# JanLohse/raw2film

Hardware: AMD Instinct MI355X
Metric: megapixels/sec full film pipeline (neg+print+grain+halation+MTF), 100MP frame (higher is better)
Workload: dtype f32 (pointwise stages, grain) + f64 (FFT stencils; the MTF's scratch images are complex64)

## Files before the change

### raw2film_amd/context.py

```python

from __future__ import annotations

import ctypes as C

import numpy as np

from . import _lib

LOG_EPS = 1e-6
LUT3D_SCALE = 0.25


class R2FError(RuntimeError):
    pass


def _host_f32(a) -> np.ndarray:
    return np.ascontiguousarray(np.asarray(a, dtype=np.float32))


class HipContext:
    def __init__(self, device: int = 0, lib_path: str | None = None):
        import torch

# ... 432 lines not shown
        self._check(self._lib.r2f_decode_u16(self._h, image_u16.data_ptr(), int(image_u16.shape[0]), int(image_u16.shape[1]),
                                             int(image_u16.shape[2]), float(np.float32(divisor)), float(np.float32(factor)),
                                             out.data_ptr(), self._stream()))
        return out

    def blit_rgba8(self, image_f32, dst_rgba, transform: dict):
        torch = self._torch
        if not (image_f32.is_cuda and image_f32.dtype == torch.float32 and image_f32.is_contiguous() and image_f32.dim() == 3
                and image_f32.shape[2] == 3):
            raise ValueError("blit_rgba8 needs a contiguous float32 (H, W, 3) CUDA tensor")
        if not (dst_rgba.is_cuda and dst_rgba.dtype == torch.uint8 and dst_rgba.is_contiguous() and dst_rgba.dim() == 3
                and dst_rgba.shape[2] == 4):
            raise ValueError("blit_rgba8 needs a contiguous uint8 (h, w, 4) CUDA destination")
        self._same_device(image_f32, "image")
        self._same_device(dst_rgba, "destination")
        t = _lib.Blit(transform["scale_x"], transform["scale_y"], transform["offset_x"], transform["offset_y"],
                      transform["canvas_min_x"], transform["canvas_min_y"], transform["canvas_max_x"], transform["canvas_max_y"],
                      (C.c_float * 3)(*transform["canvas_color"]))
        self._check(self._lib.r2f_blit_rgba8(self._h, image_f32.data_ptr(), int(image_f32.shape[0]), int(image_f32.shape[1]),
                                             dst_rgba.data_ptr(), int(dst_rgba.shape[0]), int(dst_rgba.shape[1]), C.byref(t),
                                             self._stream()))
        return dst_rgba

    def histogram_render(self, counts, mix_table, height: int, target=None):
        torch = self._torch
        mix = np.ascontiguousarray(np.asarray(mix_table, dtype=np.uint8).reshape(8, 4))
        image = torch.empty((int(height), 256, 4), dtype=torch.uint8, device=self.device)
        if not (isinstance(counts, torch.Tensor) and counts.is_cuda and counts.dtype in (torch.int32, torch.uint32)
                and tuple(counts.shape) == (3, 256)):
            raise ValueError("histogram_render needs the (3, 256) int32 CUDA counts of histogram_counts")
        self._same_device(counts, "counts")
        counts = counts.contiguous()
        if target is not None and not (target.is_cuda and target.dtype == torch.uint8 and target.is_contiguous() and target.dim() == 3
                                       and target.shape[2] == 4):
            raise ValueError("histogram_render needs a contiguous uint8 (h, w, 4) CUDA target")
        if target is not None:
            self._same_device(target, "target")
        self._check(self._lib.r2f_histogram_render(
            self._h, counts.data_ptr(), mix.ctypes.data, int(height), image.data_ptr(),
            target.data_ptr() if target is not None else None, int(target.shape[0]) if target is not None else 0,
            int(target.shape[1]) if target is not None else 0, self._stream()))
        return image

    def stencil_stats(self, which: int):
        out = (C.c_int * 24)()
        self._check(self._lib.r2f_stencil_stats(self._h, int(which), out))
        keys = ("entries", "rowsteps", "phases", "sym", "kh", "kw", "q")
        stats = []
        for c in range(3):
            d = dict(zip(keys, out[8 * c:8 * c + 7]))
            word = out[8 * c + 7]
            d["unrolled"] = (d["sym"] >> 1) & 0x7F
            d["separable"] = (d["sym"] >> 8) & 1
            d["sym"] &= 1
            d["fft"] = word & 1
            dims = (word >> 1) & 0x1FFFFFFF
            d["window"] = (dims // 4096, dims % 4096) if dims else None
            d["real_spectrum"] = (word >> 30) & 1
            stats.append(d)
        return stats

    def stream_copy(self, src, dst):
        nbytes = src.numel() * src.element_size()
        if dst.numel() * dst.element_size() != nbytes or not (src.is_cuda and dst.is_cuda and src.is_contiguous() and dst.is_contiguous()):
            raise ValueError("stream_copy needs two contiguous CUDA tensors of the same size in bytes")
        self._same_device(src, "source")
        self._same_device(dst, "destination")
        self._check(self._lib.r2f_stream_copy(self._h, src.data_ptr(), dst.data_ptr(), nbytes, self._stream()))

    def kernel_timing(self, cls: int):
        ms, n, b = C.c_double(), C.c_int(), C.c_double()
        self._check(self._lib.r2f_kernel_timing(self._h, int(cls), C.byref(ms), C.byref(n), C.byref(b)))
        return ms.value, n.value, b.value

    def histogram_counts(self, image_u8):
        torch = self._torch
        if not (image_u8.is_cuda and image_u8.dtype == torch.uint8 and image_u8.is_contiguous() and image_u8.dim() == 3
                and image_u8.shape[2] == 3):
            raise ValueError("histogram_counts needs a contiguous uint8 (H, W, 3) CUDA tensor")
        self._same_device(image_u8, "image")
        counts = torch.empty((3, 256), dtype=torch.int32, device=self.device)
        self._check(self._lib.r2f_histogram_u8(self._h, image_u8.data_ptr(), int(image_u8.shape[0]), int(image_u8.shape[1]),
                                               counts.data_ptr(), self._stream()))
        return counts

    def jpeg_bound_bytes(self, H: int, W: int, subsampling: int = 2) -> int:
        if int(subsampling) == 2:
            return int(self._lib.r2f_jpeg_bound_bytes(int(H), int(W)))
        return int(self._lib.r2f_jpeg_bound_bytes_ex(int(H), int(W), int(subsampling)))

    def jpeg_bound_bytes_opts(self, H: int, W: int, quality: int, subsampling: int = 2, optimize: bool = False,
                              progressive: bool = False) -> int:
        opts = _lib.JpegOpts(int(quality), int(subsampling), 1 if optimize else 0, 1 if progressive else 0)
        return int(self._lib.r2f_jpeg_bound_bytes_opts(C.byref(opts), int(H), int(W)))

    def jpeg_encode(self, image_u8, quality: int, subsampling: int = 2, optimize: bool = False, progressive: bool = False):
        torch = self._torch
        if not (isinstance(image_u8, torch.Tensor) and image_u8.is_cuda and image_u8.dtype == torch.uint8 and image_u8.dim() == 3
                and image_u8.shape[2] == 3 and image_u8.stride(2) == 1 and image_u8.stride(1) == 3):
            raise ValueError("jpeg_encode needs a uint8 (H, W, 3) CUDA tensor with packed pixels (row stride free)")
        self._same_device(image_u8, "image")
        H, W = int(image_u8.shape[0]), int(image_u8.shape[1])
        bound = (self.jpeg_bound_bytes_opts(H, W, quality, subsampling, optimize, True) if progressive else
                 self.jpeg_bound_bytes(H, W, subsampling))
        if bound == 0:
            raise ValueError(f"jpeg_encode: a JPEG holds 1 .. 65535 pixels per side, got {H} x {W} (subsampling {subsampling})")
# ... 56 lines not shown
```

### raw2film_amd/csrc/r2f_api.hip

```cpp
#include <hip/hip_runtime.h>

#include <cmath>
#include <cstdarg>
#include <cstdio>
#include <cstring>
#include <string>
#include <algorithm>
#include <vector>

#include "../../include/r2f.h"
#include "r2f_launch.h"
#include "r2f_jpeg.h"
#include "r2f_plan.h"

using namespace r2f;

namespace {

struct DeviceBuf {
    void* p = nullptr;
    size_t bytes = 0;
    void release() {
        if (p) (void)hipFree(p);
        p = nullptr;
// ... 33 lines not shown
    DevCurve grain_lut{};
    StencilSet stencil[3];
    struct TileOrder {
        int gx = 0, gy = 0;
        DeviceBuf buf;
    } tile_order[4];
    int tile_order_next = 0;
    static constexpr int kFftShapes = 6;
    static int fft_shape_index(int ny, int nx) { return (ny == 512 ? 3 : 0) + (nx == 256 ? 0 : (nx == 512 ? 1 : 2)); }
    DeviceBuf fft_tw, fft_kf[3][3][kFftShapes], fft_s1, fft_kimg;
    bool fft_kf_valid[3][3][kFftShapes] = {};
    int fft_kf_dims[3][3] = {{0, 0, 0}, {0, 0, 0}, {0, 0, 0}};
    int fft_last_real[3][3] = {{0, 0, 0}, {0, 0, 0}, {0, 0, 0}};
    int opt_fft_window = 0;
    int opt_fft_window_max = 512;
    int opt_fft_window_rows = 0;
    int opt_timing = 0;
    std::vector<std::pair<hipEvent_t, hipEvent_t>> timing_ev[6];
    double timing_bytes[6] = {0, 0, 0, 0, 0, 0};
    int opt_fft = 1;
    int opt_fft_min_taps = 400;
    hipStream_t fft_stream[4] = {nullptr, nullptr, nullptr, nullptr};
    hipEvent_t fft_ev_in = nullptr, fft_ev_out[4] = {nullptr, nullptr, nullptr, nullptr};
    int opt_fft_streams = 2;
    int opt_fft_even = 1;
    int opt_fft_batch = 192;
    int opt_fft_s32 = 1 << R2F_KERNEL_MTF;
    int opt_fft_s96 = 0;
    int opt_fft_s96_auto = 1;
    float curve_slope_max = 0.f;
    bool frame_dyn_armed = false;
    bool capturing = false;
    int opt_fft_epi_lds = 1;
    int opt_fft_real = 1;
    int opt_fft_mixed_sign = 1;
    int opt_fft_cols_walk = 1;
    int cu_count = 0;
    bool fft_kf_real[3][3][kFftShapes] = {};
    DeviceBuf lanczos_buf;
    DeviceBuf lanczos_f32_buf;
    int lanczos_key[4] = {0, 0, 0, 0};
    int opt_xcd_band = 0;
    int opt_variant = -1;
    int opt_xcd_remap = 2;
    int opt_ablate = 0;
    int opt_sym = 1;
    DeviceBuf grain_fixed_w;
    bool grain_fixed_valid = false;
    int grain_fixed_r = 0, grain_fixed_same = 0;
    int opt_grain_fixed = 1;
    bool grain_sep = false;
    float grain_sep_u[3][19] = {}, grain_sep_v[3][10] = {};
    int opt_grain_sep = 1;
    DeviceBuf stencil_fixed_w[3];
    bool stencil_fixed_valid[3] = {false, false, false};
    int opt_stencil_fixed = 1;
    int opt_front_fast = 1;
    int opt_front_blocks = 6;
    int opt_lds_kb = 80;
    DeviceBuf frame_buf;
    DeviceBuf range_tiles, dyn_flags;
    int tiles_tyn = 0, tiles_txn = 0;
    int dyn_flags_ppc = 0;
    struct RenderGraph {
        const void* in = nullptr;
        int in_layout = 0;
        float* out_f32 = nullptr;
        uint8_t* out_u8 = nullptr;
        int H = 0, W = 0;
        void* workspace = nullptr;
        r2f_params p{};
        hipGraph_t graph = nullptr;
        hipGraphExec_t exec = nullptr;
        hipEvent_t done = nullptr;
        uint64_t last_use = 0;
        bool never = false;
        bool dyn_armed = false;
    };
    std::vector<RenderGraph> graphs;
    struct RetiredGraph {
        hipGraph_t graph;
        hipGraphExec_t exec;
        hipEvent_t done;
    };
    std::vector<RetiredGraph> retired;
    uint64_t graphs_generation = 0;
    uint64_t graph_clock = 0;
    RenderGraph warm;
    bool warm_valid = false;
    std::vector<RenderGraph> seen;
    hipStream_t cap_stream = nullptr;
    int opt_render_graph = 1;
    uint64_t stat_replays = 0, stat_captures = 0, stat_eager = 0, stat_dropped = 0;
    DeviceBuf jpeg_scratch;
    struct JpegRows {
        bool open = false;
        int H = 0, W = 0, next_y = 0;
        int sampling = 2, header_len = 0;
        uint8_t* out = nullptr;
        uint64_t* out_len = nullptr;
    } jpeg_rows;
    DeviceBuf jpeg_carry;
    DeviceBuf jpeg_freq;
};

namespace {
// ... 691 lines not shown
        return R2F_OK;
    }
    if (!strcmp(name, "stencil_lds_kb")) {
        if (value < 8 || value > 160) return fail(ctx, R2F_EINVAL, "stencil_lds_kb must be in [8, 160]");
        ctx->opt_lds_kb = value;
        return R2F_OK;
    }
    if (!strcmp(name, "stencil_sym")) {
        ctx->opt_sym = value ? 1 : 0;
        return R2F_OK;
    }
    if (!strcmp(name, "stencil_ablate")) {
        ctx->opt_ablate = value;
        return R2F_OK;
    }
    if (!strcmp(name, "kernel_timing")) {
        ctx->opt_timing = value & 7;
        return R2F_OK;
    }
    if (!strcmp(name, "stencil_fft")) {
        ctx->opt_fft = value ? 1 : 0;
        return R2F_OK;
    }
    if (!strcmp(name, "stencil_fft_window")) {
        if (value != 0 && value != 256 && value != 512 && value != 1024) return fail(ctx, R2F_EINVAL, "stencil_fft_window must be 0, 256, 512 or 1024");
        ctx->opt_fft_window = value;
        return R2F_OK;
    }
    if (!strcmp(name, "stencil_fft_window_max")) {
        if (value != 256 && value != 512 && value != 1024) return fail(ctx, R2F_EINVAL, "stencil_fft_window_max must be 256, 512 or 1024");
        ctx->opt_fft_window_max = value;
        return R2F_OK;
    }
    if (!strcmp(name, "stencil_fft_even_batches")) {
        ctx->opt_fft_even = value ? 1 : 0;
        return R2F_OK;
    }
    if (!strcmp(name, "stencil_fixed")) {
        ctx->opt_stencil_fixed = value ? 1 : 0;
        return R2F_OK;
    }
    if (!strcmp(name, "grain_fixed")) {
        ctx->opt_grain_fixed = value ? 1 : 0;
        return R2F_OK;
    }
    if (!strcmp(name, "front_fast")) {
        ctx->opt_front_fast = value ? 1 : 0;
        return R2F_OK;
    }
    if (!strcmp(name, "grain_separable")) {
        ctx->opt_grain_sep = value ? 1 : 0;
        return R2F_OK;
    }
    if (!strcmp(name, "front_blocks_per_cu")) {
        if (value < 1 || value > 64) return fail(ctx, R2F_EINVAL, "front_blocks_per_cu must be in [1, 64]");
        ctx->opt_front_blocks = value;
        return R2F_OK;
    }
    if (!strcmp(name, "stencil_fft_window_rows")) {
        if (value != 0 && value != 256 && value != 512) return fail(ctx, R2F_EINVAL, "stencil_fft_window_rows must be 0, 256 or 512");
        ctx->opt_fft_window_rows = value;
        return R2F_OK;
    }
    if (!strcmp(name, "stencil_fft_min_taps")) {
        ctx->opt_fft_min_taps = value;
        return R2F_OK;
    }
    if (!strcmp(name, "stencil_fft_streams")) {
        if (value < 1 || value > 4) return fail(ctx, R2F_EINVAL, "stencil_fft_streams must be in [1, 4]");
        ctx->opt_fft_streams = value;
        return R2F_OK;
    }
    if (!strcmp(name, "stencil_fft_cols_walk")) {
        ctx->opt_fft_cols_walk = value ? 1 : 0;
        return R2F_OK;
    }
    if (!strcmp(name, "stencil_fft_mixed_sign")) {
        ctx->opt_fft_mixed_sign = value ? 1 : 0;
        return R2F_OK;
    }
    if (!strcmp(name, "stencil_fft_real_spectrum")) {
        ctx->opt_fft_real = value ? 1 : 0;
        return R2F_OK;
    }
    if (!strcmp(name, "stencil_fft_epilogue_lds")) {
        ctx->opt_fft_epi_lds = value ? 1 : 0;
        return R2F_OK;
    }
    if (!strcmp(name, "stencil_fft_scratch96_auto")) {
        ctx->opt_fft_s96_auto = value ? 1 : 0;
        return R2F_OK;
    }
    if (!strcmp(name, "stencil_fft_scratch96")) {
        if (value < 0 || value > 7) return fail(ctx, R2F_EINVAL, "stencil_fft_scratch96 is a mask over the three stencils (0..7)");
        ctx->opt_fft_s96 = value;
        return R2F_OK;
    }
    if (!strcmp(name, "stencil_fft_scratch32")) {
        if (value < 0 || value > 7) return fail(ctx, R2F_EINVAL, "stencil_fft_scratch32 is a mask over the three stencils (0..7)");
        ctx->opt_fft_s32 = value;
        return R2F_OK;
    }
    if (!strcmp(name, "stencil_fft_batch")) {
        if (value < 1) return fail(ctx, R2F_EINVAL, "stencil_fft_batch must be >= 1");
        ctx->opt_fft_batch = value;
        return R2F_OK;
// ... 248 lines not shown
    if (!ctx || !p) return R2F_EINVAL;
    R2F_GUARD(ctx);
    return run_stencil(ctx, R2F_KERNEL_MTF, din, dout, y0, y1, W, H_global, 0, 0.f, static_cast<hipStream_t>(stream));
}

int r2f_stage_stencil(r2f_ctx* ctx, int which, const r2f_planes* src, const r2f_planes* dst, int y0, int y1, int W,
                      int H_global, void* stream) {
    if (!ctx) return R2F_EINVAL;
    R2F_GUARD(ctx);
    if (which < 0 || which > 2) return fail(ctx, R2F_EINVAL, "stencil: which must be 0..2");
    return run_stencil(ctx, which, src, dst, y0, y1, W, H_global, 0, 0.f, static_cast<hipStream_t>(stream));
}

int r2f_kernel_timing(r2f_ctx* ctx, int cls, double* total_ms, int* launches, double* bytes) {
    if (!ctx || cls < 0 || cls > 5 || !total_ms || !launches || !bytes) return R2F_EINVAL;
    R2F_GUARD(ctx);
    double sum = 0.0;
    for (auto& ev : ctx->timing_ev[cls]) {
        R2F_HIP(ctx, hipEventSynchronize(ev.second));
        float ms = 0.f;
        R2F_HIP(ctx, hipEventElapsedTime(&ms, ev.first, ev.second));
        sum += ms;
        (void)hipEventDestroy(ev.first);
        (void)hipEventDestroy(ev.second);
    }
    *total_ms = sum;
    *launches = (int)ctx->timing_ev[cls].size();
    *bytes = ctx->timing_bytes[cls];
    ctx->timing_ev[cls].clear();
    ctx->timing_bytes[cls] = 0.0;
    return R2F_OK;
}

int r2f_stencil_stats(r2f_ctx* ctx, int which, int* out) {
    if (!ctx || !out) return R2F_EINVAL;
    R2F_GUARD(ctx);
    if (which < 0 || which > 2) return fail(ctx, R2F_EINVAL, "stencil: which must be 0..2");
    StencilSet& set = ctx->stencil[which];
    if (!set.present) return fail(ctx, R2F_EINVAL, "stencil %d not set (r2f_set_kernel)", which);
    if (!set.built_q) {
        const StencilVariant& sv = kStencilVariants[ctx->opt_variant >= 0 ? ctx->opt_variant : 0];
        int rc = ensure_stencil(ctx, which, sv.Q, sv.TW(), sv.TH(), (size_t)ctx->opt_lds_kb * 1024, which == 2);
        if (rc) return rc;
    }
    for (int c = 0; c < 3; ++c) {
        const DevStencil& d = set.dev[c];
        int* o = out + 8 * c;
        const int all[3] = {0, 1, 2};
        const int fr = which == R2F_KERNEL_GRAIN ? (ctx->opt_grain_fixed ? fixed_stencil_radius(set, all, 3, 9) : 0)
                                                 : (ctx->opt_stencil_fixed && ctx->opt_variant <= 0 && !fft_eligible(ctx, set, c)
                                                        ? fixed_stencil_radius(set, &c, 1, kFixedMaxR)
                                                        : 0);
        const int sep = which == R2F_KERNEL_GRAIN && fr && ctx->grain_fixed_valid && ctx->grain_sep && ctx->opt_grain_sep;
        o[0] = d.n_entries, o[1] = d.n_rowsteps, o[2] = d.n_phases, o[3] = d.sym | (fr << 1) | (sep << 8);
        o[4] = d.kh, o[5] = d.kw, o[6] = set.built_q;
        o[7] = fft_eligible(ctx, set, c) ? 1 | (ctx->fft_kf_dims[which][c] << 1) | (ctx->fft_last_real[which][c] << 30) : 0;
    }
    return R2F_OK;
}

static bool burn_geometry(const r2f_params* p, int H, int W, int* h_lo, int* w_lo) { return plan::burn_geometry(p->burn_cell, H, W, h_lo, w_lo); }

static int ensure_grain_fixed(r2f_ctx* ctx) {
    if (ctx->grain_fixed_valid) return R2F_OK;
    StencilSet& set = ctx->stencil[R2F_KERNEL_GRAIN];
    ctx->grain_fixed_valid = true;
    const int chans[3] = {0, 1, 2};
    ctx->grain_fixed_r = fixed_stencil_radius(set, chans, 3, 9);
    ctx->grain_sep = false;
    if (!ctx->grain_fixed_r) return R2F_OK;
    bool same = false;
    const std::vector<float> w = fixed_stencil_weights(set, ctx->grain_fixed_r, kTailQ, &same);
    ctx->grain_fixed_same = same ? 1 : 0;
    ctx->grain_sep = plan::separable_taps(taps_of(set), ctx->grain_fixed_r, ctx->grain_sep_u, ctx->grain_sep_v);
    return upload(ctx, ctx->grain_fixed_w, w.data(), w.size() * sizeof(float));
}

static int run_tail(r2f_ctx* ctx, const r2f_params* p, const r2f_planes* density, const r2f_planes* planes_out,
                    const float* burn_map, float* out_f32, uint8_t* out_u8, int out_gy0, int y0, int y1, int W, int H_global,
                    void* stream, const r2f_planes* gfield = nullptr) {
    if (y1 <= y0) return R2F_OK;
    const bool field_only = density == nullptr && planes_out != nullptr;
    if (field_only) {
        static const r2f_planes none = {nullptr, 0, 0, 0};
        density = &none;
    }
    const bool to_planes = planes_out != nullptr;
    if (W <= 0 || y0 < 0 || y1 > H_global || (!to_planes && y0 < out_gy0)) return fail(ctx, R2F_EINVAL, "tail: bad geometry");
    if (!to_planes && !out_f32 && !out_u8) return fail(ctx, R2F_EINVAL, "tail: no output buffer");
    if (!to_planes && !ctx->lut3d.tex) return fail(ctx, R2F_EINVAL, "output LUT not set (r2f_set_lut3d)");
    int rc = field_only ? R2F_OK : check_rows(ctx, "tail src", density, y0, y1);
    if (rc) return rc;
    TailArgs a;
    memset(&a, 0, sizeof a);
    a.src = to_dev(density);
    a.out_f32 = out_f32;
    a.out_u8 = out_u8;
    a.out_gy0 = out_gy0;
    a.y0 = y0;
    a.y1 = y1;
    a.W = W;
    a.H_global = H_global;
    a.grain = (p->flags & R2F_F_GRAIN) ? 1 : 0;
    if (gfield) {
        if (!a.grain) return fail(ctx, R2F_EINVAL, "tail: a grain field was passed but the grain flag is off");
        rc = check_rows(ctx, "grain field", gfield, y0, y1);
        if (rc) return rc;
// ... 6 lines not shown
    a.mono = (p->flags & R2F_F_GRAIN_MONO) ? 1 : 0;
    a.frame = static_cast<const FrameParams*>(ctx->frame_buf.p);
    a.lut3d = ctx->lut3d;
    a.lut3d_scale = p->lut3d_scale;
    a.lut3d_mode = p->lut3d_mode;
    bool vec = field_only ? true : planes_vec_ok(density, W);
    if (gfield) vec = vec && planes_vec_ok(gfield, W);
    if (to_planes) {
        if (!a.grain) return fail(ctx, R2F_EINVAL, "grain stage called with the grain flag off");
        rc = check_rows(ctx, "grain dst", planes_out, y0, y1);
        if (rc) return rc;
        if (!field_only && planes_overlap(density, planes_out, W) &&
            !(density->data == planes_out->data && density->plane_stride == planes_out->plane_stride && density->gy0 == planes_out->gy0))
            return fail(ctx, R2F_EINVAL, "grain: source and destination planes overlap without being the same buffer");
        a.to_planes = field_only ? 2 : 1;
        a.dst = to_dev(planes_out);
        vec = vec && planes_vec_ok(planes_out, W);
    } else {
        vec = vec && (!out_f32 || aligned16(out_f32)) && (!out_u8 || (reinterpret_cast<uintptr_t>(out_u8) & 3u) == 0);
        if (burn_map) {
            if (a.grain || a.has_gfield)
                return fail(ctx, R2F_EINVAL, "tail with a burn map: apply the grain first (r2f_stage_grain) and clear R2F_F_GRAIN");
            int h_lo, w_lo;
            if (!burn_geometry(p, H_global, W, &h_lo, &w_lo)) return fail(ctx, R2F_EINVAL, "burn: bad burn_cell");
            a.burn.map = burn_map;
            a.burn.h_lo = h_lo;
            a.burn.w_lo = w_lo;
            a.burn.h_up = h_lo * p->burn_cell;
            a.burn.w_up = w_lo * p->burn_cell;
            a.burn.zy = a.burn.h_up > 1 ? (double)(h_lo - 1) / (double)(a.burn.h_up - 1) : 0.0;
            a.burn.zx = a.burn.w_up > 1 ? (double)(w_lo - 1) / (double)(a.burn.w_up - 1) : 0.0;
            a.burn.strength = p->burn_strength;
        }
    }
    a.vec = vec ? 1 : 0;
    if (a.grain) {
        if (!ctx->grain_lut.cells) return fail(ctx, R2F_EINVAL, "grain LUT not set (r2f_set_grain_lut)");
        if (!ctx->stencil[R2F_KERNEL_GRAIN].present) {
            const float one = 1.f;
            rc = r2f_set_kernel(ctx, R2F_KERNEL_GRAIN, &one, 1, 1, 1);
            if (rc) return rc;
        }
        rc = ensure_stencil(ctx, R2F_KERNEL_GRAIN, kTailQ, 4 * kTailBX, kTailQ * kTailBY, 0, true);
        if (rc) return rc;
        for (int c = 0; c < 3; ++c) a.gk[c] = ctx->stencil[R2F_KERNEL_GRAIN].dev[c];
        rc = ensure_grain_fixed(ctx);
        if (rc) return rc;
        a.fixed_r = ctx->opt_grain_fixed ? ctx->grain_fixed_r : 0;
        a.fixed_same = ctx->grain_fixed_same;
        a.fixed_w = static_cast<const float*>(ctx->grain_fixed_w.p);
        a.sep = (a.fixed_r && ctx->opt_grain_sep && ctx->grain_sep && (!a.mono || ctx->grain_fixed_same)) ? 1 : 0;
        memcpy(a.sep_u, ctx->grain_sep_u, sizeof a.sep_u);
        memcpy(a.sep_v, ctx->grain_sep_v, sizeof a.sep_v);
        if (tail_lds_bytes(a.gk, a.mono) > kMaxLds)
            return fail(ctx, R2F_ETOOLARGE, "grain stencil %dx%d does not fit the LDS noise tile", a.gk[0].kh, a.gk[0].kw);
        a.grain_lut = ctx->grain_lut;
    }
    if (a.grain && !(p->flags & R2F_F_FRAME_RESIDENT)) {
        rc = write_frame_params(ctx, p, static_cast<hipStream_t>(stream), 0);
        if (rc) return rc;
    }
    R2F_HIP(ctx, launch_tail(a, static_cast<hipStream_t>(stream)));
    return R2F_OK;
}

int r2f_stage_tail(r2f_ctx* ctx, const r2f_params* p, const r2f_planes* density, const float* burn_map, float* out_f32,
                   uint8_t* out_u8, int out_gy0, int y0, int y1, int W, int H_global, void* stream) {
    if (!ctx || !p) return R2F_EINVAL;
    R2F_GUARD(ctx);
    return run_tail(ctx, p, density, nullptr, burn_map, out_f32, out_u8, out_gy0, y0, y1, W, H_global, stream);
}

int r2f_stage_grain_field(r2f_ctx* ctx, const r2f_params* p, const r2f_planes* field, int y0, int y1, int W, int H_global,
                          void* stream) {
    if (!ctx || !p) return R2F_EINVAL;
    R2F_GUARD(ctx);
    if (!field) return fail(ctx, R2F_EINVAL, "grain field: null destination");
    return run_tail(ctx, p, nullptr, field, nullptr, nullptr, nullptr, 0, y0, y1, W, H_global, stream);
}

int r2f_stage_tail_field(r2f_ctx* ctx, const r2f_params* p, const r2f_planes* density, const r2f_planes* field, float* out_f32,
                         uint8_t* out_u8, int out_gy0, int y0, int y1, int W, int H_global, void* stream) {
    if (!ctx || !p) return R2F_EINVAL;
    R2F_GUARD(ctx);
    if (!field) return fail(ctx, R2F_EINVAL, "tail: null grain field");
    return run_tail(ctx, p, density, nullptr, nullptr, out_f32, out_u8, out_gy0, y0, y1, W, H_global, stream, field);
}

int r2f_stage_grain(r2f_ctx* ctx, const r2f_params* p, const r2f_planes* din, const r2f_planes* dout, int y0, int y1, int W,
                    int H_global, void* stream) {
    if (!ctx || !p) return R2F_EINVAL;
    R2F_GUARD(ctx);
    if (!dout) return fail(ctx, R2F_EINVAL, "grain: null destination");
    return run_tail(ctx, p, din, dout, nullptr, nullptr, nullptr, 0, y0, y1, W, H_global, stream);
}

int r2f_stage_burn_sums(r2f_ctx* ctx, const r2f_params* p, const r2f_planes* density, float* cell_sums, int y0, int y1, int W,
                        int H_global, void* stream) {
    if (!ctx || !p) return R2F_EINVAL;
    R2F_GUARD(ctx);
    int h_lo, w_lo;
    if (!cell_sums || !burn_geometry(p, H_global, W, &h_lo, &w_lo)) return fail(ctx, R2F_EINVAL, "burn sums: bad arguments");
    if (y0 < 0 || y1 > H_global || y1 < y0) return fail(ctx, R2F_EINVAL, "burn sums: bad rows");
    if (y1 > y0) {
        int rc = check_rows(ctx, "burn src", density, y0, y1);
        if (rc) return rc;
// ... 728 lines not shown
```

### raw2film_amd/csrc/r2f_kernels.hip

```cpp
#include <algorithm>

#include "r2f_launch.h"

#include "../../include/r2f.h"

#ifndef R2F_CURVE_BATCH3
#define R2F_CURVE_BATCH3 1
#endif

namespace r2f {

const StencilVariant kStencilVariants[kNumStencilVariants] = {
    {0, 32, 16, 4},
    {1, 16, 8, 4},
    {2, 32, 8, 4},
};

__device__ __forceinline__ uint32_t to_u8(float v) {
    float s = fminf(fmaxf(v * 255.0f, 0.0f), 255.0f);
    return (uint32_t)s;
}

__device__ __forceinline__ void emit_hwc(float* out_f32, uint8_t* out_u8, long long orow, int x, int W, int nv, bool vec,
                                         const float (&r)[4], const float (&g)[4], const float (&b)[4]) {
// ... 546 lines not shown
        const int gy = tile_y0 + ty * Q + q;
        if (gy >= a.y1) break;
        float r[4], g[4], b[4];
        if (a.to_planes == 2) {
#pragma unroll
            for (int p = 0; p < 4; ++p) r[p] = G[0][q / 2][p][q & 1], g[p] = G[1][q / 2][p][q & 1], b[p] = G[2][q / 2][p][q & 1];
            store_planes4(a.dst, gy, gx, a.W, nv, vec, r, g, b);
            continue;
        }
#pragma unroll
        for (int p = 0; p < 4; ++p) r[p] = pre_r[q][p], g[p] = pre_g[q][p], b[p] = pre_b[q][p];
#pragma unroll
        for (int p = 0; p < 4; ++p) {
            float ar, ag, ab;
            if (R2F_CURVE_BATCH3) {
                float v3[3] = {r[p], g[p], b[p]};
                if (a.cells_in_lds)
                    curve_eval_batch<3, 3>((const float4*)cells_lds, a.grain_lut, 0, v3);
                else
                    curve_eval_batch<3, 3>(gcells, a.grain_lut, 0, v3);
                ar = v3[0], ag = v3[1], ab = v3[2];
            } else if (a.cells_in_lds) {
                ar = curve_eval_at((const float4*)cells_lds, a.grain_lut, 0, r[p]);
                ag = curve_eval_at((const float4*)cells_lds, a.grain_lut, 1, g[p]);
                ab = curve_eval_at((const float4*)cells_lds, a.grain_lut, 2, b[p]);
            } else {
                ar = curve_eval(a.grain_lut, 0, r[p]);
                ag = curve_eval(a.grain_lut, 1, g[p]);
                ab = curve_eval(a.grain_lut, 2, b[p]);
            }
            r[p] = fmaxf(__fadd_rn(r[p], __fmul_rn(G[0][q / 2][p][q & 1], ar)), 0.f);
            g[p] = fmaxf(__fadd_rn(g[p], __fmul_rn(G[1][q / 2][p][q & 1], ag)), 0.f);
            b[p] = fmaxf(__fadd_rn(b[p], __fmul_rn(G[2][q / 2][p][q & 1], ab)), 0.f);
            if (!a.to_planes && !(R2F_TAIL_EXP & 4)) {
                if (!tetra_nonneg)
                    apply_lut3d(a.lut3d, a.lut3d_scale, a.lut3d_mode, r[p], g[p], b[p]);
                else if (R2F_TAIL_LUT_BATCH == 1)
                    apply_lut3d_tetra_nonneg(a.lut3d, s3, r[p], g[p], b[p]);
                else if ((p + 1) % R2F_TAIL_LUT_BATCH == 0) {
                    constexpr int NB = R2F_TAIL_LUT_BATCH;
                    float rn[NB], gn[NB], bn[NB];
#pragma unroll
                    for (int k = 0; k < NB; ++k) rn[k] = r[p + 1 - NB + k], gn[k] = g[p + 1 - NB + k], bn[k] = b[p + 1 - NB + k];
                    apply_lut3d_tetra_nonneg_batch<NB>(a.lut3d, s3, rn, gn, bn);
#pragma unroll
                    for (int k = 0; k < NB; ++k) r[p + 1 - NB + k] = rn[k], g[p + 1 - NB + k] = gn[k], b[p + 1 - NB + k] = bn[k];
                }
            }
        }
        if (a.to_planes)
            store_planes4(a.dst, gy, gx, a.W, nv, vec, r, g, b);
        else
            emit_hwc(a.out_f32, a.out_u8, gy - a.out_gy0, gx, a.W, nv, vec, r, g, b);
    }
}

__device__ __forceinline__ void area_cell(int d, double scale, int ssize, int& s_first, int& s_last, int& s1, int& s2,
                                          double& w_first, double& w_full, double& w_last) {
    const double f1 = d * scale, f2 = f1 + scale;
    const double cell = fmin(scale, (double)ssize - f1);
    s1 = (int)ceil(f1);
    s2 = min((int)floor(f2), ssize - 1);
    s1 = min(s1, s2);
    w_first = (s1 - f1 > 1e-3) ? (s1 - f1) / cell : 0.0;
    w_full = 1.0 / cell;
    w_last = (f2 - s2 > 1e-3) ? fmin(fmin(f2 - s2, 1.0), cell) / cell : 0.0;
    s_first = max(s1 - 1, 0);
    s_last = s2;
}

__device__ __forceinline__ float area_weight(int s, int s1, int s2, double w_first, double w_full, double w_last) {
    if (s == s1 - 1) return (float)w_first;
    if (s >= s1 && s < s2) return (float)w_full;
    if (s == s2) return (float)w_last;
    return 0.f;
}

__global__ __launch_bounds__(256) void burn_sums_kernel(const BurnSumsArgs a) {
    const int j = blockIdx.x, i = blockIdx.y;
    int ry0, ry1, rs1, rs2, cx0, cx1, cs1, cs2;
    double wyf, wy, wyl, wxf, wx, wxl;
    area_cell(i, (double)a.H_global / a.h_lo, a.H_global, ry0, ry1, rs1, rs2, wyf, wy, wyl);
    area_cell(j, (double)a.W / a.w_lo, a.W, cx0, cx1, cs1, cs2, wxf, wx, wxl);
    const int ra = max(ry0, a.y0), rb = min(ry1, a.y1 - 1);
    const int ncols = cx1 - cx0 + 1;
    const float* green = a.src.data + a.src.plane_stride;
    double acc = 0.0;
    if (rb >= ra) {
        const int n = (rb - ra + 1) * ncols;
        for (int idx = threadIdx.x; idx < n; idx += 256) {
            const int rr = idx / ncols, cc = idx - rr * ncols;
            const int y = ra + rr, x = cx0 + cc;
            const float w = area_weight(y, rs1, rs2, wyf, wy, wyl) * area_weight(x, cs1, cs2, wxf, wx, wxl);
            acc += (double)w * (double)green[(long long)(y - a.src.gy0) * a.W + x];
        }
    }
    __shared__ double red[256];
    red[threadIdx.x] = acc;
    __syncthreads();
    for (int s = 128; s > 0; s >>= 1) {
        if (threadIdx.x < s) red[threadIdx.x] += red[threadIdx.x + s];
        __syncthreads();
    }
    if (threadIdx.x == 0) a.cell_sums[i * a.w_lo + j] = (float)red[0];
}

// ... 371 lines not shown
    if (ldsc) {
        int gy = ((a.blocks_per_cu > 0 ? a.blocks_per_cu : 6) * 256 + gx - 1) / gx;
        if (gy > row_groups) gy = row_groups;
        if (gy < 1) gy = 1;
        launch_k(front_kernel<true>, dim3(gx, gy), block, cell_bytes, s, a);
    } else {
        launch_k(front_kernel<false>, dim3(gx, row_groups), block, 0, s, a);
    }
    return take_launch_status();
}

hipError_t launch_stencil(const StencilArgs& a, int variant, hipStream_t s) {
    if (a.y1 <= a.y0 || a.W <= 0) return hipSuccess;
    const StencilVariant& v = kStencilVariants[variant];
    const size_t lds = stencil_lds_bytes(v, a.st, 3);
    dim3 block(v.BX * v.BY), grid((a.W + v.TW() - 1) / v.TW(), (a.y1 - a.y0 + v.TH() - 1) / v.TH(), a.nchan);
    if (variant == 0 && a.fixed_r > 0) {
#define R2F_STENCIL_FIXED(R)                                                                        \
    case R:                                                                                        \
        if (a.epilogue == 1)                                                                       \
            launch_k((stencil_kernel<32, 16, 4, 1, R>), grid, block, lds, s, a);         \
        else                                                                                       \
            launch_k((stencil_kernel<32, 16, 4, 0, R>), grid, block, lds, s, a);         \
        return take_launch_status();
        switch (a.fixed_r) {
            R2F_STENCIL_FIXED(1)
            R2F_STENCIL_FIXED(2)
            R2F_STENCIL_FIXED(3)
            R2F_STENCIL_FIXED(4)
            R2F_STENCIL_FIXED(5)
            R2F_STENCIL_FIXED(6)
            R2F_STENCIL_FIXED(7)
            R2F_STENCIL_FIXED(8)
            R2F_STENCIL_FIXED(9)
            R2F_STENCIL_FIXED(10)
            R2F_STENCIL_FIXED(11)
            default:
                break;
        }
#undef R2F_STENCIL_FIXED
    }
    const int key = variant * 2 + (a.epilogue == 1 ? 1 : 0);
    switch (key) {
        case 0: launch_k((stencil_kernel<32, 16, 4, 0>), grid, block, lds, s, a); break;
        case 1: launch_k((stencil_kernel<32, 16, 4, 1>), grid, block, lds, s, a); break;
        case 2: launch_k((stencil_kernel<16, 8, 4, 0>), grid, block, lds, s, a); break;
        case 3: launch_k((stencil_kernel<16, 8, 4, 1>), grid, block, lds, s, a); break;
        case 4: launch_k((stencil_kernel<32, 8, 4, 0>), grid, block, lds, s, a); break;
        default: launch_k((stencil_kernel<32, 8, 4, 1>), grid, block, lds, s, a); break;
    }
    return take_launch_status();
}

hipError_t launch_tail(const TailArgs& a, hipStream_t s) {
    if (a.y1 <= a.y0 || a.W <= 0) return hipSuccess;
    if (!a.grain) {
        Lut3dArgs l;
        l.src = a.src;
        l.out_f32 = a.out_f32;
        l.out_u8 = a.out_u8;
        l.out_gy0 = a.out_gy0;
        l.y0 = a.y0;
        l.y1 = a.y1;
        l.W = a.W;
        l.lut3d = a.lut3d;
        l.lut3d_scale = a.lut3d_scale;
        l.lut3d_mode = a.lut3d_mode;
        l.vec = a.vec;
        l.burn = a.burn;
        l.gfield = a.gfield;
        l.has_gfield = a.has_gfield;
        l.grain_lut = a.grain_lut;
        const int quads = (a.W + 3) / 4;
        dim3 block(64, 4), grid((quads + 63) / 64, (a.y1 - a.y0 + 3) / 4);
        launch_k(lut3d_kernel, grid, block, 0, s, l);
        return take_launch_status();
    }
    const int TW = 4 * kTailBX, TH = kTailQ * kTailBY;
    dim3 block(kTailBX * kTailBY), grid((a.W + TW - 1) / TW, (a.y1 - a.y0 + TH - 1) / TH);
    TailArgs b = a;
    b.cells_off = (int)tail_plane_floats(a.gk, a.mono);
    b.cells_in_lds = tail_lds_bytes(a.gk, a.mono, 1, a.grain_lut.m) <= 80 * 1024 ? 1 : 0;
    const size_t lds = tail_lds_bytes(a.gk, a.mono, b.cells_in_lds, a.grain_lut.m);
    switch (a.fixed_r) {
#define R2F_TAIL_FIXED(R)                                                        \
    case R:                                                                     \
        if (a.sep)                                                              \
            launch_k((tail_kernel<R, true>), grid, block, lds, s, b); \
        else                                                                    \
            launch_k((tail_kernel<R>), grid, block, lds, s, b);       \
        break;
        R2F_TAIL_FIXED(1)
        R2F_TAIL_FIXED(2)
        R2F_TAIL_FIXED(3)
        R2F_TAIL_FIXED(4)
        R2F_TAIL_FIXED(5)
        R2F_TAIL_FIXED(6)
        R2F_TAIL_FIXED(7)
        R2F_TAIL_FIXED(8)
        R2F_TAIL_FIXED(9)
#undef R2F_TAIL_FIXED
        default:
            launch_k((tail_kernel<0>), grid, block, lds, s, b);
            break;
    }
    return take_launch_status();
}

hipError_t launch_burn_sums(const BurnSumsArgs& a, hipStream_t s) {
    if (a.h_lo <= 0 || a.w_lo <= 0) return hipSuccess;
    launch_k(burn_sums_kernel, dim3(a.w_lo, a.h_lo), dim3(256), 0, s, a);
    return take_launch_status();
}

hipError_t launch_burn_map(const BurnMapArgs& a, hipStream_t s) {
    launch_k(burn_map_kernel, dim3(1), dim3(256), 0, s, a);
    return take_launch_status();
}

hipError_t launch_chroma_h(const ChromaArgs& a, hipStream_t s) {
    if (a.y1 <= a.y0 || a.W <= 0) return hipSuccess;
    launch_k(chroma_h_kernel, dim3((a.W + kChromaSeg - 1) / kChromaSeg, a.y1 - a.y0), dim3(256), 0, s, a);
    return take_launch_status();
}

hipError_t launch_chroma_v(const ChromaArgs& a, hipStream_t s) {
    if (a.y1 <= a.y0 || a.W <= 0) return hipSuccess;
    const int quads = (a.W + 3) / 4;
    launch_k(chroma_v_kernel, dim3((quads + 63) / 64, (a.y1 - a.y0 + 3) / 4), dim3(64, 4), 0, s, a);
    return take_launch_status();
}

hipError_t launch_resize_area(const ResizeArgs& a, hipStream_t s) {
// ... 111 lines not shown
```

### raw2film_amd/csrc/r2f_launch.h

```cpp
#pragma once

#include <cstdint>
#include <tuple>
#include <type_traits>
#include "r2f_device.h"

struct r2f_blit;

namespace r2f {

inline thread_local hipError_t tl_launch_error = hipSuccess;
template <typename... KArgs, typename... Args>
inline void launch_k(void (*kernel)(KArgs...), dim3 grid, dim3 block, size_t lds, hipStream_t s, const Args&... args) {
    static_assert(sizeof...(KArgs) == sizeof...(Args), "one value per kernel parameter");
    std::tuple<std::remove_cv_t<KArgs>...> vals{static_cast<std::remove_cv_t<KArgs>>(args)...};
    void* ptrs[sizeof...(KArgs)];
    int i = 0;
    std::apply([&](auto&... v) { ((ptrs[i++] = static_cast<void*>(&v)), ...); }, vals);
    const hipError_t e = hipLaunchKernel(reinterpret_cast<const void*>(kernel), grid, block, ptrs, lds, s);
    if (e != hipSuccess) {
        (void)hipGetLastError();
        if (tl_launch_error == hipSuccess) tl_launch_error = e;
    }
}
// ... 51 lines not shown
    int fixed_r;
    const float* fixed_w;
};

struct BurnUp {
    const float* map;
    int h_lo, w_lo;
    int h_up, w_up;
    double zy, zx;
    float strength;
};

struct BurnSumsArgs {
    DevPlanes src;
    float* cell_sums;
    int y0, y1, W, H_global;
    int h_lo, w_lo;
};

struct BurnMapArgs {
    const float* cell_sums;
    float* map;
    float* scratch;
    int h_lo, w_lo;
    float d_ref;
    double w[13];
};

struct TailArgs {
    DevPlanes src;
    float* out_f32;
    uint8_t* out_u8;
    int out_gy0;
    int y0, y1, W, H_global;
    int grain;
    int to_planes;
    DevPlanes dst;
    BurnUp burn;
    int mono;
    const FrameParams* frame;
    DevStencil gk[3];
    DevCurve grain_lut;
    DevLut3D lut3d;
    float lut3d_scale;
    int lut3d_mode;
    int vec;
    int cells_in_lds, cells_off;
    DevPlanes gfield;
    int has_gfield;
    int fixed_r, fixed_same;
    const float* fixed_w;
    int sep;
    float sep_u[3][19], sep_v[3][10];
};

constexpr int kChromaMaxTaps = 63;
struct ChromaArgs {
    const void* in;
    int in_layout, in_gy0, in_rows;
    DevPlanes src;
    DevPlanes dst;
    int y0, y1, W, H_global;
    int radius;
    int vec;
    float w[kChromaMaxTaps];
};

struct ResizeArgs {
    const void* in;
    int in_layout, H, W;
    DevPlanes dst;
    int out_h, out_w;
};

struct WarpArgs {
    const void* in;
    int in_layout, H, W;
    DevPlanes dst;
    int out_h, out_w, oy, ox;
    float m[6];
};

struct LanczosArgs {
    const uint8_t* src;
    uint8_t* dst;
    int H, W, out_h, out_w;
    const int* xofs;
    const short* xcoef;
    const int* yofs;
    const short* ycoef;
};

struct TapArgs {
    DevPlanes src, dst;
    int ch, y0, y1, W;
    float w;
    int epilogue;
    DevCurve curve;
    float log_eps;
    int vec;
};
hipError_t launch_single_tap(const TapArgs& a, hipStream_t s);

constexpr int kFftN = 256;
struct FftConvArgs {
    DevPlanes src, dst;
// ... 16 lines not shown
    int cols_walk;
    int cols_slots;
    double2* s1;
    int s32;
    const int* dyn_flags;
    int epilogue;
    DevCurve curve;
    float log_eps;
    int vec4;
    int epi_lds;
    int epi_lds_off;
};
hipError_t fft_init_attributes();
hipError_t launch_fft_rows_fwd(const FftConvArgs& a, hipStream_t s);
hipError_t launch_fft_cols(const FftConvArgs& a, int mode, hipStream_t s);
hipError_t launch_fft_rows_inv(const FftConvArgs& a, hipStream_t s);
hipError_t launch_fft_decide(const FftConvArgs& a, const RangeRecord& rec, float bound, float floor_, int* flags, hipStream_t s);

struct NoiseArgs {
    uint32_t* hash;
    float* noise;
    int y0, y1, W;
    const FrameParams* frame;
    int mono;
};

struct StencilVariant {
    int id;
    int BX, BY, Q;
    int TW() const { return 4 * BX; }
    int TH() const { return Q * BY; }
};
constexpr int kNumStencilVariants = 3;
extern const StencilVariant kStencilVariants[kNumStencilVariants];
#ifndef R2F_TAIL_BX
#define R2F_TAIL_BX 16
#endif
#ifndef R2F_TAIL_BY
#define R2F_TAIL_BY 32
#endif
#ifndef R2F_TAIL_Q
#define R2F_TAIL_Q 2
#endif
constexpr int kTailBX = R2F_TAIL_BX, kTailBY = R2F_TAIL_BY, kTailQ = R2F_TAIL_Q;
constexpr size_t kMaxLds = 160 * 1024;

size_t stencil_lds_bytes(const StencilVariant& v, const DevStencil* st, int nchan);
size_t tail_lds_bytes(const DevStencil* gk, int mono, int cells_in_lds = 0, int grain_m = 2);

hipError_t init_kernel_attributes();
hipError_t launch_front(const FrontArgs& a, hipStream_t s);
hipError_t launch_stencil(const StencilArgs& a, int variant, hipStream_t s);
hipError_t launch_tail(const TailArgs& a, hipStream_t s);
hipError_t launch_warp_affine(const WarpArgs& a, hipStream_t s);
hipError_t launch_lanczos4_u8(const LanczosArgs& a, hipStream_t s);
hipError_t launch_noise(const NoiseArgs& a, hipStream_t s);
hipError_t launch_frame_params(const RangeRecord& rec, const FrameParams& v, int mode, hipStream_t s);
hipError_t launch_exposure_range(const DevPlanes& src, int y0, int y1, int y2, int y3, int W, int mask, const RangeRecord& rec, hipStream_t s);

hipError_t launch_histogram_u8(const uint8_t* image, long long n_bytes, uint32_t* counts, hipStream_t s);
hipError_t launch_burn_sums(const BurnSumsArgs& a, hipStream_t s);
hipError_t launch_resize_area_u8(const uint8_t* src, int H, int W, uint8_t* dst, int out_h, int out_w, hipStream_t s);
hipError_t launch_stream_copy(const void* src, void* dst, long long bytes, hipStream_t s);
hipError_t launch_decode_u16(const uint16_t* src, long long n, int ch, float divisor, float factor, float* dst, hipStream_t s);
hipError_t launch_lanczos4_f32(const void* in, int in_layout, int H, int W, const DevPlanes& dst, int out_h, int out_w, const int* xofs,
                               const float* xcoef, const int* yofs, const float* ycoef, hipStream_t s);
hipError_t launch_blit_rgba8(const float* src, int H, int W, uint8_t* dst, int dst_h, int dst_w, const ::r2f_blit& t, hipStream_t s);
hipError_t launch_histogram_render(const uint32_t* counts, const uint8_t* mix_rgba, int height, uint8_t* image, uint8_t* target, int th,
                                   int tw, hipStream_t s);
hipError_t launch_burn_map(const BurnMapArgs& a, hipStream_t s);
hipError_t launch_chroma_h(const ChromaArgs& a, hipStream_t s);
hipError_t launch_chroma_v(const ChromaArgs& a, hipStream_t s);
hipError_t launch_resize_area(const ResizeArgs& a, hipStream_t s);

}
```

Measured before the change: 20870.

## Add wave-strip grain tail kernel using DPP lane shifts instead of LDS tile

Adds a new tail kernel form for separable grain stencils with radius up to 4. Each wave walks down a 128-pixel-wide strip, two pixels per lane. It generates noise in registers, builds the horizontal taps with DPP row shifts plus readlane halos, and keeps the vertical window in a rolling register buffer, so the LDS noise tile is no longer needed. The new form is the automatic default, with a knob to pick either form. It trades shared-memory traffic and barriers for more registers and serial row walking, and DPP row_shl/shr only move data within 16-lane rows, which makes correctness at row boundaries subtle.

```diff
diff --git a/raw2film_amd/context.py b/raw2film_amd/context.py
--- a/raw2film_amd/context.py
+++ b/raw2film_amd/context.py
@@ -508,6 +508,7 @@
             word = out[8 * c + 7]
             d["unrolled"] = (d["sym"] >> 1) & 0x7F
             d["separable"] = (d["sym"] >> 8) & 1
+            d["strip"] = (d["sym"] >> 9) & 1
             d["sym"] &= 1
             d["fft"] = word & 1
             dims = (word >> 1) & 0x1FFFFFFF
diff --git a/raw2film_amd/csrc/r2f_api.hip b/raw2film_amd/csrc/r2f_api.hip
--- a/raw2film_amd/csrc/r2f_api.hip
+++ b/raw2film_amd/csrc/r2f_api.hip
@@ -109,6 +109,7 @@
     bool grain_sep = false;
     float grain_sep_u[3][19] = {}, grain_sep_v[3][10] = {};
     int opt_grain_sep = 1;
+    int opt_tail_form = 0;
     DeviceBuf stencil_fixed_w[3];
     bool stencil_fixed_valid[3] = {false, false, false};
     int opt_stencil_fixed = 1;
@@ -906,6 +907,11 @@
         ctx->opt_grain_sep = value ? 1 : 0;
         return R2F_OK;
     }
+    if (!strcmp(name, "tail_form")) {
+        if (value < 0 || value > 2) return fail(ctx, R2F_EINVAL, "tail_form must be 0 (automatic), 1 (LDS tile) or 2 (wave strip)");
+        ctx->opt_tail_form = value;
+        return R2F_OK;
+    }
     if (!strcmp(name, "front_blocks_per_cu")) {
         if (value < 1 || value > 64) return fail(ctx, R2F_EINVAL, "front_blocks_per_cu must be in [1, 64]");
         ctx->opt_front_blocks = value;
@@ -1260,7 +1266,8 @@
                                                         ? fixed_stencil_radius(set, &c, 1, kFixedMaxR)
                                                         : 0);
         const int sep = which == R2F_KERNEL_GRAIN && fr && ctx->grain_fixed_valid && ctx->grain_sep && ctx->opt_grain_sep;
-        o[0] = d.n_entries, o[1] = d.n_rowsteps, o[2] = d.n_phases, o[3] = d.sym | (fr << 1) | (sep << 8);
+        const int strip = sep && fr <= 4 && (ctx->opt_tail_form ? ctx->opt_tail_form : kTailAutoForm) == 2;
+        o[0] = d.n_entries, o[1] = d.n_rowsteps, o[2] = d.n_phases, o[3] = d.sym | (fr << 1) | (sep << 8) | (strip << 9);
         o[4] = d.kh, o[5] = d.kw, o[6] = set.built_q;
         o[7] = fft_eligible(ctx, set, c) ? 1 | (ctx->fft_kf_dims[which][c] << 1) | (ctx->fft_last_real[which][c] << 30) : 0;
     }
@@ -1373,6 +1380,7 @@
         a.sep = (a.fixed_r && ctx->opt_grain_sep && ctx->grain_sep && (!a.mono || ctx->grain_fixed_same)) ? 1 : 0;
         memcpy(a.sep_u, ctx->grain_sep_u, sizeof a.sep_u);
         memcpy(a.sep_v, ctx->grain_sep_v, sizeof a.sep_v);
+        a.form = ctx->opt_tail_form;
         if (tail_lds_bytes(a.gk, a.mono) > kMaxLds)
             return fail(ctx, R2F_ETOOLARGE, "grain stencil %dx%d does not fit the LDS noise tile", a.gk[0].kh, a.gk[0].kw);
         a.grain_lut = ctx->grain_lut;
diff --git a/raw2film_amd/csrc/r2f_kernels.hip b/raw2film_amd/csrc/r2f_kernels.hip
--- a/raw2film_amd/csrc/r2f_kernels.hip
+++ b/raw2film_amd/csrc/r2f_kernels.hip
@@ -622,6 +622,176 @@
             store_planes4(a.dst, gy, gx, a.W, nv, vec, r, g, b);
         else
             emit_hwc(a.out_f32, a.out_u8, gy - a.out_gy0, gx, a.W, nv, vec, r, g, b);
+    }
+}
+
+#ifndef R2F_STRIP_LUT_BATCH
+#define R2F_STRIP_LUT_BATCH 2
+#endif
+constexpr int kStripW = 128, kStripH = 64, kStripWaves = 4;
+
+__device__ __forceinline__ float dpp_from_left(float edge, float v) {
+    return __builtin_bit_cast(float, __builtin_amdgcn_update_dpp(__builtin_bit_cast(int, edge), __builtin_bit_cast(int, v), 0x138, 0xf, 0xf, false));
+}
+__device__ __forceinline__ float dpp_from_right(float edge, float v) {
+    return __builtin_bit_cast(float, __builtin_amdgcn_update_dpp(__builtin_bit_cast(int, edge), __builtin_bit_cast(int, v), 0x130, 0xf, 0xf, false));
+}
+__device__ __forceinline__ float lane_value(float v, int lane) {
+    return __builtin_bit_cast(float, __builtin_amdgcn_readlane(__builtin_bit_cast(int, v), lane));
+}
+
+template <int R, bool MONO>
+__global__ __launch_bounds__(64 * kStripWaves) void tail_strip_kernel(const TailArgs a) {
+    extern __shared__ __attribute__((aligned(16))) float smem[];
+    static_assert(R >= 1 && R <= 4, "two lanes to either side hold the taps of a pixel pair");
+    constexpr int NCH = MONO ? 1 : 3;
+    const float4* gcells = a.grain_lut.cells;
+    float4* cells_lds = reinterpret_cast<float4*>(smem);
+    if (a.cells_in_lds) {
+        for (int i = threadIdx.x; i < 3 * (a.grain_lut.m - 1); i += 64 * kStripWaves) cells_lds[i] = gcells[i];
+        __syncthreads();
+    }
+    const int lane = threadIdx.x & 63;
+    const int x0 = (blockIdx.x * kStripWaves + (int)(threadIdx.x >> 6)) * kStripW;
+    const int ys = a.y0 + blockIdx.y * kStripH, ye = min(ys + kStripH, a.y1);
+    if (x0 >= a.W || ys >= ye) return;
+    const uint32_t seed = a.frame->seed;
+    const int X = x0 + 2 * lane;
+    const bool inside = X < a.W;
+    const uint32_t sx0 = (uint32_t)clampi(X, 0, a.W - 1), sx1 = (uint32_t)clampi(X + 1, 0, a.W - 1);
+    const int hrow = lane >> 3, hc = lane & 7;
+    const uint32_t hsx = (uint32_t)clampi(hc < 4 ? x0 - 4 + hc : x0 + kStripW - 4 + hc, 0, a.W - 1);
+    const float s3 = a.lut3d_scale * (float)(a.lut3d.n - 1);
+
+    float win[NCH][2][2 * R];
+#pragma unroll
+    for (int c = 0; c < NCH; ++c)
+#pragma unroll
+        for (int i = 0; i < 2 * R; ++i) win[c][0][i] = win[c][1][i] = 0.f;
+    float halo[3] = {0.f, 0.f, 0.f};
+
+    const int t0 = ys - R;
+    for (int t = t0; t < ye + R; ++t) {
+        const int y = t - R;
+        float dr[2] = {0.f, 0.f}, dg[2] = {0.f, 0.f}, db[2] = {0.f, 0.f};
+        if (y >= ys && inside) {
+            const float* p0 = a.src.data + (long long)(y - a.src.gy0) * a.W + X;
+            const float* p1 = p0 + a.src.plane_stride;
+            const float* p2 = p1 + a.src.plane_stride;
+            const float2v v0 = __builtin_nontemporal_load(reinterpret_cast<const float2v*>(p0));
+            const float2v v1 = __builtin_nontemporal_load(reinterpret_cast<const float2v*>(p1));
+            const float2v v2 = __builtin_nontemporal_load(reinterpret_cast<const float2v*>(p2));
+            dr[0] = v0.x, dr[1] = v0.y, dg[0] = v1.x, dg[1] = v1.y, db[0] = v2.x, db[1] = v2.y;
+        }
+        const int blk = (t - t0) & 7;
+        if (blk == 0 && !(R2F_TAIL_EXP & 1)) {
+            const uint32_t sy = (uint32_t)clampi(t + hrow, 0, a.H_global - 1);
+            gaussian_noise(hsx, sy, seed, MONO, halo[0], halo[1], halo[2]);
+        }
+        float n[3][2] = {{0.f, 0.f}, {0.f, 0.f}, {0.f, 0.f}};
+        if (!(R2F_TAIL_EXP & 1)) {
+            const uint32_t sy = (uint32_t)clampi(t, 0, a.H_global - 1);
+            gaussian_noise(sx0, sy, seed, MONO, n[0][0], n[1][0], n[2][0]);
+            gaussian_noise(sx1, sy, seed, MONO, n[0][1], n[1][1], n[2][1]);
+#pragma unroll
+            for (int c = 0; c < NCH; ++c) asm volatile("" : "+v"(n[c][0]), "+v"(n[c][1]));
+        }
+        float G[3][2];
+#pragma unroll
+        for (int c = 0; c < NCH; ++c) {
+            float s[10];
+            s[4] = n[c][0], s[5] = n[c][1];
+            s[2] = dpp_from_left(lane_value(halo[c], 8 * blk + 2), s[4]);
+            s[3] = dpp_from_left(lane_value(halo[c], 8 * blk + 3), s[5]);
+            s[6] = dpp_from_right(lane_value(halo[c], 8 * blk + 4), s[4]);
+            s[7] = dpp_from_right(lane_value(halo[c], 8 * blk + 5), s[5]);
+            if (R > 2) {
+                s[0] = dpp_from_left(lane_value(halo[c], 8 * blk + 0), s[2]);
+                s[1] = dpp_from_left(lane_value(halo[c], 8 * blk + 1), s[3]);
+                s[8] = dpp_from_right(lane_value(halo[c], 8 * blk + 6), s[6]);
+                s[9] = dpp_from_right(lane_value(halo[c], 8 * blk + 7), s[7]);
+            } else {
+                s[0] = s[1] = s[8] = s[9] = 0.f;
+            }
+            const float* wv = a.sep_v[c];
+            const float* wu = a.sep_u[c];
+#pragma unroll
+            for (int p = 0; p < 2; ++p) {
+                float acc = wv[0] * (s[4 + p - R] + s[4 + p + R]);
+#pragma unroll
+                for (int j = 1; j < R; ++j) acc = fmaf(wv[j], s[4 + p - R + j] + s[4 + p + R - j], acc);
+                const float h = fmaf(wv[R], s[4 + p], acc);
+                float g = 0.f;
+#pragma unroll
+                for (int i = 0; i < 2 * R; ++i) g = fmaf(wu[i], win[c][p][i], g);
+                G[c][p] = fmaf(wu[2 * R], h, g);
+#pragma unroll
+                for (int i = 0; i + 1 < 2 * R; ++i) win[c][p][i] = win[c][p][i + 1];
+                win[c][p][2 * R - 1] = h;
+            }
+        }
+        if (y < ys || !inside) continue;
+        if (R2F_TAIL_EXP & 2) {
+#pragma unroll
+            for (int c = 0; c < NCH; ++c) G[c][0] = G[c][1] = 0.f;
+        }
+        if (MONO) {
+#pragma unroll
+            for (int p = 0; p < 2; ++p) G[1][p] = G[2][p] = G[0][p];
+        }
+#pragma unroll
+        for (int p = 0; p < 2; ++p) {
+            float ar, ag, ab;
+            if (R2F_CURVE_BATCH3) {
+                float v3[3] = {dr[p], dg[p], db[p]};
+                if (a.cells_in_lds)
+                    curve_eval_batch<3, 3>((const float4*)cells_lds, a.grain_lut, 0, v3);
+                else
+                    curve_eval_batch<3, 3>(gcells, a.grain_lut, 0, v3);
+                ar = v3[0], ag = v3[1], ab = v3[2];
+            } else if (a.cells_in_lds) {
+                ar = curve_eval_at((const float4*)cells_lds, a.grain_lut, 0, dr[p]);
+                ag = curve_eval_at((const float4*)cells_lds, a.grain_lut, 1, dg[p]);
+                ab = curve_eval_at((const float4*)cells_lds, a.grain_lut, 2, db[p]);
+            } else {
+                ar = curve_eval(a.grain_lut, 0, dr[p]);
+                ag = curve_eval(a.grain_lut, 1, dg[p]);
+                ab = curve_eval(a.grain_lut, 2, db[p]);
+            }
+            dr[p] = fmaxf(__fadd_rn(dr[p], __fmul_rn(G[0][p], ar)), 0.f);
+            dg[p] = fmaxf(__fadd_rn(dg[p], __fmul_rn(G[1][p], ag)), 0.f);
+            db[p] = fmaxf(__fadd_rn(db[p], __fmul_rn(G[2][p], ab)), 0.f);
+        }
+        if (a.to_planes) {
+            float* p0 = a.dst.data + (long long)(y - a.dst.gy0) * a.W + X;
+            float* p1 = p0 + a.dst.plane_stride;
+            float* p2 = p1 + a.dst.plane_stride;
+            *reinterpret_cast<float2v*>(p0) = (float2v){dr[0], dr[1]};
+            *reinterpret_cast<float2v*>(p1) = (float2v){dg[0], dg[1]};
+            *reinterpret_cast<float2v*>(p2) = (float2v){db[0], db[1]};
+            continue;
+        }
+        if (!(R2F_TAIL_EXP & 4)) {
+            if (R2F_STRIP_LUT_BATCH == 2) {
+                apply_lut3d_tetra_nonneg_batch<2>(a.lut3d, s3, dr, dg, db);
+            } else {
+#pragma unroll
+                for (int p = 0; p < 2; ++p) apply_lut3d_tetra_nonneg(a.lut3d, s3, dr[p], dg[p], db[p]);
+            }
+        }
+        const long long base = ((long long)(y - a.out_gy0) * a.W + X) * 3;
+        if (a.out_f32) {
+            float2v* o = reinterpret_cast<float2v*>(a.out_f32 + base);
+            o[0] = (float2v){dr[0], dg[0]};
+            o[1] = (float2v){db[0], dr[1]};
+            o[2] = (float2v){dg[1], db[1]};
+        }
+        if (a.out_u8) {
+            uint16_t* o = reinterpret_cast<uint16_t*>(a.out_u8 + base);
+            o[0] = (uint16_t)(to_u8(dr[0]) | (to_u8(dg[0]) << 8));
+            o[1] = (uint16_t)(to_u8(db[0]) | (to_u8(dr[1]) << 8));
+            o[2] = (uint16_t)(to_u8(dg[1]) | (to_u8(db[1]) << 8));
+        }
     }
 }
 
@@ -1099,6 +1269,13 @@
     return take_launch_status();
 }
 
+bool tail_takes_strip_form(const TailArgs& a) {
+    const int form = a.form ? a.form : kTailAutoForm;
+    const bool tetra_nonneg = a.lut3d_mode == 0 && a.lut3d.n >= 2 && a.lut3d.n <= 512;
+    return form == 2 && a.grain && a.sep && a.fixed_r >= 1 && a.fixed_r <= 4 && a.vec && a.to_planes != 2 &&
+           (a.to_planes == 1 || tetra_nonneg) && (!a.mono || a.fixed_same);
+}
+
 hipError_t launch_tail(const TailArgs& a, hipStream_t s) {
     if (a.y1 <= a.y0 || a.W <= 0) return hipSuccess;
     if (!a.grain) {
@@ -1123,9 +1300,32 @@
         launch_k(lut3d_kernel, grid, block, 0, s, l);
         return take_launch_status();
     }
+    TailArgs b = a;
+    if (tail_takes_strip_form(a)) {
+        const size_t cell_bytes = (size_t)3 * (a.grain_lut.m - 1) * sizeof(float4);
+        b.cells_in_lds = cell_bytes <= 48 * 1024 ? 1 : 0;
+        b.cells_off = 0;
+        const size_t lds = b.cells_in_lds ? cell_bytes : 0;
+        const int SW = kStripW * kStripWaves;
+        dim3 block(64 * kStripWaves), grid((a.W + SW - 1) / SW, (a.y1 - a.y0 + kStripH - 1) / kStripH);
+        switch (a.fixed_r) {
+#define R2F_TAIL_STRIP(R)                                                          \
+    case R:                                                                        \
+        if (a.mono)                                                                \
+            launch_k((tail_strip_kernel<R, true>), grid, block, lds, s, b);  \
+        else                                                                       \
+            launch_k((tail_strip_kernel<R, false>), grid, block, lds, s, b); \
+        break;
+            R2F_TAIL_STRIP(1)
+            R2F_TAIL_STRIP(2)
+            R2F_TAIL_STRIP(3)
+            R2F_TAIL_STRIP(4)
+#undef R2F_TAIL_STRIP
+        }
+        return take_launch_status();
+    }
     const int TW = 4 * kTailBX, TH = kTailQ * kTailBY;
     dim3 block(kTailBX * kTailBY), grid((a.W + TW - 1) / TW, (a.y1 - a.y0 + TH - 1) / TH);
-    TailArgs b = a;
     b.cells_off = (int)tail_plane_floats(a.gk, a.mono);
     b.cells_in_lds = tail_lds_bytes(a.gk, a.mono, 1, a.grain_lut.m) <= 80 * 1024 ? 1 : 0;
     const size_t lds = tail_lds_bytes(a.gk, a.mono, b.cells_in_lds, a.grain_lut.m);
diff --git a/raw2film_amd/csrc/r2f_launch.h b/raw2film_amd/csrc/r2f_launch.h
--- a/raw2film_amd/csrc/r2f_launch.h
+++ b/raw2film_amd/csrc/r2f_launch.h
@@ -127,6 +127,7 @@
     const float* fixed_w;
     int sep;
     float sep_u[3][19], sep_v[3][10];
+    int form;
 };
 
 constexpr int kChromaMaxTaps = 63;
@@ -249,6 +250,8 @@
 hipError_t launch_front(const FrontArgs& a, hipStream_t s);
 hipError_t launch_stencil(const StencilArgs& a, int variant, hipStream_t s);
 hipError_t launch_tail(const TailArgs& a, hipStream_t s);
+constexpr int kTailAutoForm = 2;
+bool tail_takes_strip_form(const TailArgs& a);
 hipError_t launch_warp_affine(const WarpArgs& a, hipStream_t s);
 hipError_t launch_lanczos4_u8(const LanczosArgs& a, hipStream_t s);
 hipError_t launch_noise(const NoiseArgs& a, hipStream_t s);
```

New measurement: 20880, median of 5. No clear change (+0.1%).
